# zxhuang1698/ShapeClipper

Measured on AMD Instinct MI355X. Metric: train-step images/sec (Pix3D cfg, bs32/GPU), higher is better.
Workload: dtype f32 (bf16x3-split MFMA, fp32 accumulate)

## Files before the change

### shapeclipper_amd/csrc/bn_act.hip

```cpp
#include <hip/hip_runtime.h>
#include <stdlib.h>
#include <stdint.h>
#include <type_traits>

namespace sc {

constexpr int BN_T = 256;

template <int W> struct Vec;
template <> struct Vec<4> {
    float v[4];
    __device__ __forceinline__ static Vec ld(const float* p) {
        const float4 t = *reinterpret_cast<const float4*>(p);
        return Vec{{t.x, t.y, t.z, t.w}};
    }
    __device__ __forceinline__ void st(float* p) const { *reinterpret_cast<float4*>(p) = make_float4(v[0], v[1], v[2], v[3]); }
};
template <> struct Vec<1> {
    float v[1];
    __device__ __forceinline__ static Vec ld(const float* p) { return Vec{{*p}}; }
    __device__ __forceinline__ void st(float* p) const { *p = v[0]; }
};

struct BnShare {
    int g, s, S, n0, Ng;
};
__device__ __forceinline__ BnShare bn_share(int N, int G) {
    BnShare sh;
    sh.S = gridDim.y / G;
    sh.g = blockIdx.y / sh.S;
    sh.s = blockIdx.y - sh.g * sh.S;
    sh.Ng = N / G;
    sh.n0 = sh.g * sh.Ng;
    return sh;
}

template <class F>
__device__ __forceinline__ void bn_iterate(const BnShare& sh, int C, int HW, int c, F&& f) {
    const int cnt = (sh.Ng - sh.s + sh.S - 1) / sh.S;
    if ((HW & 3) == 0) {
        const int hw4 = HW >> 2, total = cnt * hw4;
#pragma unroll 2
        for (int idx = threadIdx.x; idx < total; idx += BN_T) {
            const int nl = idx / hw4, i = idx - nl * hw4;
            f(((size_t)(sh.n0 + sh.s + nl * sh.S) * C + c) * HW + 4 * i, std::integral_constant<int, 4>{});
        }
    } else {
        const int total = cnt * HW;
        for (int idx = threadIdx.x; idx < total; idx += BN_T) {
            const int nl = idx / HW, i = idx - nl * HW;
            f(((size_t)(sh.n0 + sh.s + nl * sh.S) * C + c) * HW + i, std::integral_constant<int, 1>{});
        }
    }
}

__device__ __forceinline__ void block_sum2(float& a, float& b, float* red) {
    for (int d = 32; d >= 1; d >>= 1) {
        a += __shfl_xor(a, d);
        b += __shfl_xor(b, d);
    }
    const int w = threadIdx.x >> 6;
    __syncthreads();
    if ((threadIdx.x & 63) == 0) {
        red[w] = a;
        red[BN_T / 64 + w] = b;
    }
    __syncthreads();
    a = 0.f;
    b = 0.f;
    for (int k = 0; k < BN_T / 64; ++k) {
        a += red[k];
        b += red[BN_T / 64 + k];
    }
}

__device__ __forceinline__ void combine_partials(const float* partial, int c, int g, int S, int G, float& a, float& b) {
    a = 0.f;
    b = 0.f;
    const float* p = partial + ((size_t)c * G * S + (size_t)g * S) * 2;
    for (int k = 0; k < S; ++k) {
        a += p[2 * k];
        b += p[2 * k + 1];
    }
}

__device__ __forceinline__ void store_partial(float* partial, int c, const BnShare& sh, int G, float a, float b) {
    float* p = partial + ((size_t)c * G * sh.S + (size_t)sh.g * sh.S + sh.s) * 2;
    p[0] = a;
    p[1] = b;
}

__global__ __launch_bounds__(BN_T) void bn_stats_kernel(const float* __restrict__ x, int N, int C, int HW, int G,
                                                        float* __restrict__ partial) {
    __shared__ float red[2 * BN_T / 64];
    const int c = blockIdx.x;
    const BnShare sh = bn_share(N, G);
    const float K = x[((size_t)sh.n0 * C + c) * HW];
    float s1 = 0.f, s2 = 0.f;
    bn_iterate(sh, C, HW, c, [&](size_t off, auto w) {
        const auto v = Vec<decltype(w)::value>::ld(x + off);
#pragma unroll
        for (int k = 0; k < decltype(w)::value; ++k) {
            const float d = v.v[k] - K;
            s1 += d;
            s2 += d * d;
        }
    });
    block_sum2(s1, s2, red);
    if (threadIdx.x == 0) store_partial(partial, c, sh, G, s1, s2);
}

struct BnStatArgs {
    const float* x; const float* partial;
    float* save_mean; float* save_rstd;
    float* run_mean; float* run_var; int64_t* n_tracked;
    int N, C, HW, G, training;
    float eps, momentum;
};

__device__ __forceinline__ void bn_forward_stats(const BnStatArgs& a, int c, const BnShare& sh, float& mean, float& rstd) {
    const float n = (float)sh.Ng * (float)a.HW;
    auto group_stats = [&](int g, float& m, float& var) {
        float s1, s2;
        combine_partials(a.partial, c, g, sh.S, a.G, s1, s2);
        const float dm = s1 / n;
        const float v0 = s2 / n - dm * dm;
        var = v0 < 0.f ? 0.f : v0;
        m = a.x[((size_t)g * sh.Ng * a.C + c) * a.HW] + dm;
    };
    if (a.training) {
        float var;
        group_stats(sh.g, mean, var);
        rstd = rsqrtf(var + a.eps);
    } else {
        mean = a.run_mean[c];
        rstd = rsqrtf(a.run_var[c] + a.eps);
    }
    if (blockIdx.y == 0 && threadIdx.x == 0) {
        for (int g = 0; g < a.G; ++g) {
            float m = mean, r = rstd;
            if (a.training) {
                float var;
                group_stats(g, m, var);
                r = rsqrtf(var + a.eps);
                if (a.run_mean) {
                    a.run_mean[c] = (1.f - a.momentum) * a.run_mean[c] + a.momentum * m;
                    a.run_var[c] = (1.f - a.momentum) * a.run_var[c] + a.momentum * (n > 1.f ? var * n / (n - 1.f) : var);
                }
            }
            a.save_mean[(size_t)g * a.C + c] = m;
            a.save_rstd[(size_t)g * a.C + c] = r;
        }
        if (a.training && a.n_tracked && c == 0) *a.n_tracked += a.G;
    }
}

struct BnFwdArgs {
    BnStatArgs st;
    const float* res; const float* gamma; const float* beta; float* y;
    int relu;
};

__global__ __launch_bounds__(BN_T) void bn_apply_fwd_kernel(BnFwdArgs a) {
    const int c = blockIdx.x;
    const BnShare sh = bn_share(a.st.N, a.st.G);
    float mean, rstd;
    bn_forward_stats(a.st, c, sh, mean, rstd);
    const float scale = a.gamma[c] * rstd, shift = a.beta[c] - mean * scale;
    const float* x = a.st.x;
    bn_iterate(sh, a.st.C, a.st.HW, c, [&](size_t off, auto w) {
        constexpr int W = decltype(w)::value;
        auto v = Vec<W>::ld(x + off);
        if (a.res) {
            const auto r = Vec<W>::ld(a.res + off);
#pragma unroll
            for (int k = 0; k < W; ++k) v.v[k] = fmaf(v.v[k], scale, shift) + r.v[k];
        } else {
#pragma unroll
            for (int k = 0; k < W; ++k) v.v[k] = fmaf(v.v[k], scale, shift);
        }
        if (a.relu) {
#pragma unroll
            for (int k = 0; k < W; ++k) v.v[k] = v.v[k] < 0.f ? 0.f : v.v[k];
        }
        v.st(a.y + off);
    });
}

struct BnBwdArgs {
    const float* dy; const float* x; const float* y;
    const float* gamma; const float* beta; const float* mean; const float* rstd;
    float* partial; float* dx; float* dres; float* dgamma; float* dbeta;
    int N, C, HW, G, relu, training, has_res;
};

template <int W>
__device__ __forceinline__ Vec<W> bn_masked_grad(const BnBwdArgs& a, size_t off, const Vec<W>& xv, float scale, float shift) {
    auto g = Vec<W>::ld(a.dy + off);
    if (a.relu) {
        if (a.has_res) {
            const auto yv = Vec<W>::ld(a.y + off);
#pragma unroll
            for (int k = 0; k < W; ++k) g.v[k] = yv.v[k] <= 0.f ? 0.f : g.v[k];
        } else {
#pragma unroll
            for (int k = 0; k < W; ++k) g.v[k] = fmaf(xv.v[k], scale, shift) <= 0.f ? 0.f : g.v[k];
        }
    }
    return g;
}

__global__ __launch_bounds__(BN_T) void bn_bwd_stats_kernel(BnBwdArgs a) {
    __shared__ float red[2 * BN_T / 64];
    const int c = blockIdx.x;
    const BnShare sh = bn_share(a.N, a.G);
    const float mean = a.mean[(size_t)sh.g * a.C + c], rstd = a.rstd[(size_t)sh.g * a.C + c];
    const float scale = a.gamma[c] * rstd, shift = a.beta[c] - mean * scale;
    float s1 = 0.f, s2 = 0.f;
    bn_iterate(sh, a.C, a.HW, c, [&](size_t off, auto w) {
        constexpr int W = decltype(w)::value;
        const auto xv = Vec<W>::ld(a.x + off);
        const auto g = bn_masked_grad<W>(a, off, xv, scale, shift);
#pragma unroll
        for (int k = 0; k < W; ++k) {
            s1 += g.v[k];
            s2 += g.v[k] * ((xv.v[k] - mean) * rstd);
        }
        if (a.dres) g.st(a.dres + off);
    });
    block_sum2(s1, s2, red);
    if (threadIdx.x == 0) store_partial(a.partial, c, sh, a.G, s1, s2);
}

__global__ __launch_bounds__(BN_T) void bn_bwd_apply_kernel(BnBwdArgs a) {
    const int c = blockIdx.x;
    const BnShare sh = bn_share(a.N, a.G);
    const float mean = a.mean[(size_t)sh.g * a.C + c], rstd = a.rstd[(size_t)sh.g * a.C + c], gamma = a.gamma[c];
    const float scale = gamma * rstd, shift = a.beta[c] - mean * scale;
    float sg, sgx;
    combine_partials(a.partial, c, sh.g, sh.S, a.G, sg, sgx);
    if (blockIdx.y == 0 && threadIdx.x == 0) {
        float tg = 0.f, tgx = 0.f;
        for (int g = 0; g < a.G; ++g) {
            float u, v;
            combine_partials(a.partial, c, g, sh.S, a.G, u, v);
            tg += u;
            tgx += v;
        }
        a.dgamma[c] = tgx;
        a.dbeta[c] = tg;
    }
    if (!a.dx) return;
    const float n = (float)sh.Ng * (float)a.HW;
    const float mg = a.training ? sg / n : 0.f, mgx = a.training ? sgx / n : 0.f;
    bn_iterate(sh, a.C, a.HW, c, [&](size_t off, auto w) {
        constexpr int W = decltype(w)::value;
        const auto xv = Vec<W>::ld(a.x + off);
        const auto g = a.dres ? Vec<W>::ld(a.dres + off) : bn_masked_grad<W>(a, off, xv, scale, shift);
        Vec<W> o;
#pragma unroll
        for (int k = 0; k < W; ++k) o.v[k] = scale * (g.v[k] - mg - (xv.v[k] - mean) * rstd * mgx);
        o.st(a.dx + off);
    });
}

struct PoolFwdArgs {
    BnStatArgs st;
    const float* gamma; const float* beta; float* y; int* idx;
    int H, W, Ho, Wo;
};

__global__ __launch_bounds__(BN_T) void bn_relu_pool_fwd_kernel(PoolFwdArgs a) {
    const int c = blockIdx.x;
    const BnShare sh = bn_share(a.st.N, a.st.G);
    const int HW = a.H * a.W, C = a.st.C;
    float mean, rstd;
    bn_forward_stats(a.st, c, sh, mean, rstd);
    const float scale = a.gamma[c] * rstd, shift = a.beta[c] - mean * scale;
    const int HoWo = a.Ho * a.Wo;
    const int cnt = (sh.Ng - sh.s + sh.S - 1) / sh.S, total = cnt * HoWo;
    for (int t = threadIdx.x; t < total; t += BN_T) {
        const int nl = t / HoWo, o = t - nl * HoWo;
        const int ho = o / a.Wo, wo = o - ho * a.Wo;
        const size_t plane = ((size_t)(sh.n0 + sh.s + nl * sh.S) * C + c);
        const float* xp = a.st.x + plane * HW;
        float best = -__builtin_inff();
        int bi = -1;
#pragma unroll
        for (int dh = 0; dh < 3; ++dh) {
            const int h = 2 * ho - 1 + dh;
            if (h < 0 || h >= a.H) continue;
#pragma unroll
            for (int dw = 0; dw < 3; ++dw) {
                const int w = 2 * wo - 1 + dw;
                if (w < 0 || w >= a.W) continue;
                const float u = fmaf(xp[h * a.W + w], scale, shift), v = u < 0.f ? 0.f : u;
                if (v > best || bi < 0 || v != v) {
                    best = v;
                    bi = h * a.W + w;
                }
            }
        }
        a.y[plane * HoWo + o] = best;
        a.idx[plane * HoWo + o] = bi;
    }
}

__global__ __launch_bounds__(BN_T) void bn_relu_pool_fwd2_kernel(PoolFwdArgs a) {
    const int c = blockIdx.x;
    const BnShare sh = bn_share(a.st.N, a.st.G);
    const int HW = a.H * a.W, C = a.st.C, W = a.W;
    float mean, rstd;
    bn_forward_stats(a.st, c, sh, mean, rstd);
    const float scale = a.gamma[c] * rstd, shift = a.beta[c] - mean * scale;
    const int HoWo = a.Ho * a.Wo;
    const int cnt = (sh.Ng - sh.s + sh.S - 1) / sh.S, total = cnt * HoWo;
    const int lane = threadIdx.x & 63;
    for (int t0 = 0; t0 < total; t0 += BN_T) {
        const int t = t0 + threadIdx.x;
        const bool on = t < total;
        const int tt = on ? t : total - 1;
        const int nl = tt / HoWo, o = tt - nl * HoWo;
        const int ho = o / a.Wo, wo = o - ho * a.Wo;
        const size_t plane = ((size_t)(sh.n0 + sh.s + nl * sh.S) * C + c);
        const float* xp = a.st.x + plane * HW;
        float best = -__builtin_inff();
        int bi = -1;
#pragma unroll
        for (int dh = 0; dh < 3; ++dh) {
            const int h = 2 * ho - 1 + dh;
            const bool hv = h >= 0 && h < a.H;
            float2 v = make_float2(0.f, 0.f);
            if (hv) v = *reinterpret_cast<const float2*>(xp + h * W + 2 * wo);
            const float u0 = fmaf(v.x, scale, shift), u1 = fmaf(v.y, scale, shift);
            const float r0 = u0 < 0.f ? 0.f : u0, r1 = u1 < 0.f ? 0.f : u1;
            float left = __shfl_up(r1, 1);
            if (lane == 0 && wo > 0 && hv) {
                const float ul = fmaf(xp[h * W + 2 * wo - 1], scale, shift);
                left = ul < 0.f ? 0.f : ul;
            }
            if (!hv) continue;
            if (wo > 0 && (left > best || bi < 0 || left != left)) { best = left; bi = h * W + 2 * wo - 1; }
            if (r0 > best || bi < 0 || r0 != r0) { best = r0; bi = h * W + 2 * wo; }
            if (r1 > best || bi < 0 || r1 != r1) { best = r1; bi = h * W + 2 * wo + 1; }
        }
        if (on) {
            a.y[plane * HoWo + o] = best;
            a.idx[plane * HoWo + o] = bi;
        }
    }
}

template <int R>
__global__ __launch_bounds__(BN_T) void bn_relu_pool_fwd_rows_kernel(PoolFwdArgs a) {
    const int c = blockIdx.x;
    const BnShare sh = bn_share(a.st.N, a.st.G);
    const int HW = a.H * a.W, C = a.st.C, W = a.W;
    float mean, rstd;
    bn_forward_stats(a.st, c, sh, mean, rstd);
    const float scale = a.gamma[c] * rstd, shift = a.beta[c] - mean * scale;
    const int HoWo = a.Ho * a.Wo;
    const int RG = (a.Ho + R - 1) / R, per = RG * a.Wo;
    const int cnt = (sh.Ng - sh.s + sh.S - 1) / sh.S, total = cnt * per;
    const int lane = threadIdx.x & 63;
    for (int t0 = 0; t0 < total; t0 += BN_T) {
        const int t = t0 + threadIdx.x;
        const bool on = t < total;
        const int tt = on ? t : total - 1;
        const int nl = tt / per, o = tt - nl * per;
        const int rg = o / a.Wo, wo = o - rg * a.Wo;
        const int ho0 = rg * R;
        const size_t plane = ((size_t)(sh.n0 + sh.s + nl * sh.S) * C + c);
        const float* xp = a.st.x + plane * HW;
        float2 v[2 * R + 1];
        float lf[2 * R + 1];
#pragma unroll
        for (int k = 0; k < 2 * R + 1; ++k) {
            const int h = 2 * ho0 - 1 + k;
            const bool hv = h >= 0 && h < a.H;
            v[k] = make_float2(0.f, 0.f);
            lf[k] = 0.f;
            if (hv) v[k] = *reinterpret_cast<const float2*>(xp + h * W + 2 * wo);
            if (lane == 0 && wo > 0 && hv) lf[k] = xp[h * W + 2 * wo - 1];
        }
        float r0[2 * R + 1], r1[2 * R + 1], left[2 * R + 1];
#pragma unroll
        for (int k = 0; k < 2 * R + 1; ++k) {
            const float u0 = fmaf(v[k].x, scale, shift), u1 = fmaf(v[k].y, scale, shift);
            r0[k] = u0 < 0.f ? 0.f : u0;
            r1[k] = u1 < 0.f ? 0.f : u1;
            left[k] = __shfl_up(r1[k], 1);
            if (lane == 0) {
                const float ul = fmaf(lf[k], scale, shift);
                left[k] = ul < 0.f ? 0.f : ul;
            }
        }
#pragma unroll
        for (int r = 0; r < R; ++r) {
            const int ho = ho0 + r;
            float best = -__builtin_inff();
            int bi = -1;
#pragma unroll
            for (int dh = 0; dh < 3; ++dh) {
                const int k = 2 * r + dh, h = 2 * ho - 1 + dh;
                if (h < 0 || h >= a.H) continue;
                if (wo > 0 && (left[k] > best || bi < 0 || left[k] != left[k])) { best = left[k]; bi = h * W + 2 * wo - 1; }
                if (r0[k] > best || bi < 0 || r0[k] != r0[k]) { best = r0[k]; bi = h * W + 2 * wo; }
                if (r1[k] > best || bi < 0 || r1[k] != r1[k]) { best = r1[k]; bi = h * W + 2 * wo + 1; }
            }
            if (on && ho < a.Ho) {
                a.y[plane * HoWo + ho * a.Wo + wo] = best;
                a.idx[plane * HoWo + ho * a.Wo + wo] = bi;
            }
        }
    }
}

struct PoolBwdArgs {
    const float* dy; const int* idx; const float* x; const float* gamma; const float* beta; const float* mean;
    const float* rstd; float* partial; float* dx;
    int N, C, H, W, Ho, Wo, G;
    float* dgamma; float* dbeta;
    int training;
};

template <bool V2, int MODE>
__global__ __launch_bounds__(BN_T) void bn_relu_pool_bwd_gather_kernel(PoolBwdArgs a) {
    __shared__ float red[2 * BN_T / 64];
    const int c = blockIdx.x;
    const BnShare sh = bn_share(a.N, a.G);
    const int HW = a.H * a.W, HoWo = a.Ho * a.Wo;
    const int Hq = (a.H + 1) >> 1, Wq = (a.W + 1) >> 1, Q = Hq * Wq;
    const float mean = a.mean[(size_t)sh.g * a.C + c], rstd = a.rstd[(size_t)sh.g * a.C + c];
    const float scale = a.gamma[c] * rstd, shift = a.beta[c] - mean * scale;
    float sg = 0.f, sgx = 0.f;
    float mg = 0.f, mgx = 0.f;
    if (MODE == 2) {
        float tsg, tsgx;
        combine_partials(a.partial, c, sh.g, sh.S, a.G, tsg, tsgx);
        if (blockIdx.y == 0 && threadIdx.x == 0) {
            float tg = 0.f, tgx = 0.f;
            for (int g = 0; g < a.G; ++g) {
                float u, v;
                combine_partials(a.partial, c, g, sh.S, a.G, u, v);
                tg += u;
                tgx += v;
            }
            a.dgamma[c] = tgx;
            a.dbeta[c] = tg;
        }
        const float n = (float)sh.Ng * (float)HW;
        mg = a.training ? tsg / n : 0.f;
        mgx = a.training ? tsgx / n : 0.f;
    }
    const int cnt = (sh.Ng - sh.s + sh.S - 1) / sh.S, total = cnt * Q;
    for (int t = threadIdx.x; t < total; t += BN_T) {
        const int nl = t / Q, q = t - nl * Q;
        const int i = q / Wq, j = q - i * Wq;
        const size_t plane = ((size_t)(sh.n0 + sh.s + nl * sh.S) * a.C + c);
        int wi[2][2];
        float wd[2][2];
#pragma unroll
        for (int di = 0; di < 2; ++di)
#pragma unroll
            for (int dj = 0; dj < 2; ++dj) {
                const bool ok = (i + di) < a.Ho && (j + dj) < a.Wo;
                const size_t o = plane * HoWo + (size_t)(i + di) * a.Wo + (j + dj);
                wi[di][dj] = ok ? a.idx[o] : -1;
                wd[di][dj] = ok ? a.dy[o] : 0.f;
            }
#pragma unroll
        for (int eh = 0; eh < 2; ++eh) {
            const int h = 2 * i + eh;
            if (h >= a.H) continue;
            float2 xrow = make_float2(0.f, 0.f), grow;
            if (V2) xrow = *reinterpret_cast<const float2*>(a.x + plane * HW + h * a.W + 2 * j);
#pragma unroll
            for (int ew = 0; ew < 2; ++ew) {
                const int w = 2 * j + ew;
                if (w >= a.W) continue;
                const int pos = h * a.W + w;
                const float xv = V2 ? (ew ? xrow.y : xrow.x) : a.x[plane * HW + pos];
                float g = 0.f;
#pragma unroll
                for (int di = 0; di <= eh; ++di)
#pragma unroll
                    for (int dj = 0; dj <= ew; ++dj)
                        if (wi[di][dj] == pos) g += wd[di][dj];
                if (!(fmaf(xv, scale, shift) > 0.f)) g = 0.f;
                const float o = MODE == 2 ? scale * (g - mg - (xv - mean) * rstd * mgx) : g;
                if (V2) { if (ew) grow.y = o; else grow.x = o; }
                else if (MODE != 1) a.dx[plane * HW + pos] = o;
                sg += g;
                sgx += g * ((xv - mean) * rstd);
            }
            if (V2 && MODE != 1) *reinterpret_cast<float2*>(a.dx + plane * HW + h * a.W + 2 * j) = grow;
        }
    }
    if (MODE == 2) return;
    block_sum2(sg, sgx, red);
    if (threadIdx.x == 0) store_partial(a.partial, c, sh, a.G, sg, sgx);
}

template <int MODE, int R>
__global__ __launch_bounds__(BN_T) void bn_relu_pool_bwd_rows_kernel(PoolBwdArgs a) {
    __shared__ float red[2 * BN_T / 64];
    const int c = blockIdx.x;
    const BnShare sh = bn_share(a.N, a.G);
    const int HW = a.H * a.W, HoWo = a.Ho * a.Wo;
    const int Hq = (a.H + 1) >> 1, Wq = a.W >> 1, RG = (Hq + R - 1) / R, Q = RG * Wq;
    const float mean = a.mean[(size_t)sh.g * a.C + c], rstd = a.rstd[(size_t)sh.g * a.C + c];
    const float scale = a.gamma[c] * rstd, shift = a.beta[c] - mean * scale;
    float sg = 0.f, sgx = 0.f;
    float mg = 0.f, mgx = 0.f;
    if (MODE == 2) {
        float tsg, tsgx;
        combine_partials(a.partial, c, sh.g, sh.S, a.G, tsg, tsgx);
        if (blockIdx.y == 0 && threadIdx.x == 0) {
            float tg = 0.f, tgx = 0.f;
            for (int g = 0; g < a.G; ++g) {
                float u, v;
                combine_partials(a.partial, c, g, sh.S, a.G, u, v);
                tg += u;
                tgx += v;
            }
            a.dgamma[c] = tgx;
            a.dbeta[c] = tg;
        }
        const float n = (float)sh.Ng * (float)HW;
        mg = a.training ? tsg / n : 0.f;
        mgx = a.training ? tsgx / n : 0.f;
    }
    const int cnt = (sh.Ng - sh.s + sh.S - 1) / sh.S, total = cnt * Q;
    const int lane = threadIdx.x & 63;
    for (int t0 = 0; t0 < total; t0 += BN_T) {
        const int t = t0 + threadIdx.x;
        const bool on = t < total;
        const int tt = on ? t : total - 1;
        const int nl = tt / Q, q = tt - nl * Q;
        const int rg = q / Wq, j = q - rg * Wq, i0 = rg * R;
        const size_t plane = ((size_t)(sh.n0 + sh.s + nl * sh.S) * a.C + c);
        int wi[R + 1][2];
        float wd[R + 1][2];
        float2 xrow[2 * R];
        const bool own_right = lane == 63 && (j + 1) < a.Wo;
#pragma unroll
        for (int di = 0; di <= R; ++di) {
            const bool okr = (i0 + di) < a.Ho;
            const size_t o = plane * HoWo + (size_t)(i0 + di) * a.Wo + j;
            wi[di][0] = okr && j < a.Wo ? a.idx[o] : -1;
            wd[di][0] = okr && j < a.Wo ? a.dy[o] : 0.f;
            wi[di][1] = okr && own_right ? a.idx[o + 1] : -1;
            wd[di][1] = okr && own_right ? a.dy[o + 1] : 0.f;
        }
#pragma unroll
        for (int k = 0; k < 2 * R; ++k) {
            const int h = 2 * i0 + k;
            xrow[k] = h < a.H ? *reinterpret_cast<const float2*>(a.x + plane * HW + h * a.W + 2 * j) : make_float2(0.f, 0.f);
        }
#pragma unroll
        for (int di = 0; di <= R; ++di) {
            const int ri = __shfl_down(wi[di][0], 1);
            const float rd = __shfl_down(wd[di][0], 1);
            if (lane != 63) {
                const bool okc = (j + 1) < a.Wo;
                wi[di][1] = okc ? ri : -1;
                wd[di][1] = okc ? rd : 0.f;
            }
        }
#pragma unroll
        for (int r = 0; r < R; ++r) {
#pragma unroll
            for (int eh = 0; eh < 2; ++eh) {
                const int h = 2 * (i0 + r) + eh;
                if (h >= a.H) continue;
                float2 grow;
#pragma unroll
                for (int ew = 0; ew < 2; ++ew) {
                    const int pos = h * a.W + 2 * j + ew;
                    const float xv = ew ? xrow[2 * r + eh].y : xrow[2 * r + eh].x;
                    float g = 0.f;
#pragma unroll
                    for (int di = 0; di <= eh; ++di)
#pragma unroll
                        for (int dj = 0; dj <= ew; ++dj)
                            if (wi[r + di][dj] == pos) g += wd[r + di][dj];
                    if (!(fmaf(xv, scale, shift) > 0.f)) g = 0.f;
                    const float o = MODE == 2 ? scale * (g - mg - (xv - mean) * rstd * mgx) : g;
                    if (ew) grow.y = o; else grow.x = o;
                    if (on) {
                        sg += g;
                        sgx += g * ((xv - mean) * rstd);
                    }
                }
                if (MODE == 2 && on) *reinterpret_cast<float2*>(a.dx + plane * HW + h * a.W + 2 * j) = grow;
            }
        }
    }
    if (MODE == 2) return;
    block_sum2(sg, sgx, red);
    if (threadIdx.x == 0) store_partial(a.partial, c, sh, a.G, sg, sgx);
}

constexpr int BNF_T = 512, BNF_V = 10, BNF_G = 4;

template <int NV>
__device__ __forceinline__ void block_sum_f(float (&v)[NV], float* red) {
#pragma unroll
    for (int k = 0; k < NV; ++k)
        for (int d = 32; d >= 1; d >>= 1) v[k] += __shfl_xor(v[k], d);
    const int w = threadIdx.x >> 6;
    __syncthreads();
    if ((threadIdx.x & 63) == 0) {
#pragma unroll
        for (int k = 0; k < NV; ++k) red[k * (BNF_T / 64) + w] = v[k];
    }
    __syncthreads();
#pragma unroll
    for (int k = 0; k < NV; ++k) {
        float t = 0.f;
        for (int j = 0; j < BNF_T / 64; ++j) t += red[k * (BNF_T / 64) + j];
        v[k] = t;
    }
}

template <int W>
__device__ __forceinline__ bool bnf_slot(int j, int N, int C, int HW, int Ng, int c, size_t& off, int& g) {
    const int per = HW / W, idx = threadIdx.x + j * BNF_T;
    if (idx >= N * per) return false;
    const int n = idx / per, i = idx - n * per;
    off = ((size_t)n * C + c) * HW + (size_t)W * i;
    g = n / Ng;
    return true;
}

template <int W>
__global__ __launch_bounds__(BNF_T) void bn_fused_fwd_kernel(BnFwdArgs a) {
    __shared__ float red[2 * BNF_G * BNF_T / 64];
    const int c = blockIdx.x, C = a.st.C, HW = a.st.HW, G = a.st.G, N = a.st.N, Ng = N / G;
    const float n = (float)Ng * (float)HW;
    const float* x = a.st.x;
    const float gamma = a.gamma[c], beta = a.beta[c];
    Vec<W> xv[BNF_V];
    size_t off[BNF_V];
    int grp[BNF_V];
#pragma unroll
    for (int j = 0; j < BNF_V; ++j) {
        grp[j] = -1;
        if (bnf_slot<W>(j, N, C, HW, Ng, c, off[j], grp[j])) xv[j] = Vec<W>::ld(x + off[j]);
    }
    float mean[BNF_G], rstd[BNF_G];
    if (a.st.training) {
        float K[BNF_G], s[2 * BNF_G];
#pragma unroll
        for (int g = 0; g < BNF_G; ++g) {
            K[g] = g < G ? x[((size_t)g * Ng * C + c) * HW] : 0.f;
            s[2 * g] = 0.f;
            s[2 * g + 1] = 0.f;
        }
#pragma unroll
        for (int j = 0; j < BNF_V; ++j)
#pragma unroll
            for (int g = 0; g < BNF_G; ++g)
                if (grp[j] == g) {
#pragma unroll
                    for (int k = 0; k < W; ++k) {
                        const float d = xv[j].v[k] - K[g];
                        s[2 * g] += d;
                        s[2 * g + 1] += d * d;
                    }
                }
        block_sum_f(s, red);
#pragma unroll
        for (int g = 0; g < BNF_G; ++g) {
            const float dm = s[2 * g] / n, v0 = s[2 * g + 1] / n - dm * dm;
            const float var = v0 < 0.f ? 0.f : v0;
            mean[g] = K[g] + dm;
            rstd[g] = rsqrtf(var + a.st.eps);
            if (g < G && threadIdx.x == 0 && a.st.run_mean) {
                a.st.run_mean[c] = (1.f - a.st.momentum) * a.st.run_mean[c] + a.st.momentum * mean[g];
                a.st.run_var[c] = (1.f - a.st.momentum) * a.st.run_var[c] + a.st.momentum * (n > 1.f ? var * n / (n - 1.f) : var);
            }
        }
    } else {
#pragma unroll
        for (int g = 0; g < BNF_G; ++g) {
            mean[g] = a.st.run_mean[c];
            rstd[g] = rsqrtf(a.st.run_var[c] + a.st.eps);
        }
    }
    if (threadIdx.x == 0) {
        for (int g = 0; g < G; ++g) {
            a.st.save_mean[(size_t)g * C + c] = mean[g < BNF_G ? g : 0];
            a.st.save_rstd[(size_t)g * C + c] = rstd[g < BNF_G ? g : 0];
        }
        if (a.st.training && a.st.n_tracked && c == 0) *a.st.n_tracked += G;
    }
#pragma unroll
    for (int j = 0; j < BNF_V; ++j) {
        if (grp[j] < 0) continue;
        float m = mean[0], r = rstd[0];
#pragma unroll
        for (int g = 1; g < BNF_G; ++g)
            if (grp[j] == g) { m = mean[g]; r = rstd[g]; }
        const float scale = gamma * r, shift = beta - m * scale;
        Vec<W> v = xv[j];
        if (a.res) {
            const auto rv = Vec<W>::ld(a.res + off[j]);
#pragma unroll
            for (int k = 0; k < W; ++k) v.v[k] = fmaf(v.v[k], scale, shift) + rv.v[k];
        } else {
#pragma unroll
            for (int k = 0; k < W; ++k) v.v[k] = fmaf(v.v[k], scale, shift);
        }
        if (a.relu) {
#pragma unroll
            for (int k = 0; k < W; ++k) v.v[k] = v.v[k] < 0.f ? 0.f : v.v[k];
        }
        v.st(a.y + off[j]);
    }
}

template <int W>
__global__ __launch_bounds__(BNF_T) void bn_fused_bwd_kernel(BnBwdArgs a) {
    __shared__ float red[2 * BNF_G * BNF_T / 64];
    const int c = blockIdx.x, C = a.C, HW = a.HW, G = a.G, N = a.N, Ng = N / G;
    const float n = (float)Ng * (float)HW;
    const float gamma = a.gamma[c], beta = a.beta[c];
    float mean[BNF_G], rstd[BNF_G];
#pragma unroll
    for (int g = 0; g < BNF_G; ++g) {
        mean[g] = a.mean[(size_t)(g < G ? g : 0) * C + c];
        rstd[g] = a.rstd[(size_t)(g < G ? g : 0) * C + c];
    }
    Vec<W> xh[BNF_V], gr[BNF_V];
    size_t off[BNF_V];
    int grp[BNF_V];
    float s[2 * BNF_G];
#pragma unroll
    for (int g = 0; g < 2 * BNF_G; ++g) s[g] = 0.f;
#pragma unroll
    for (int j = 0; j < BNF_V; ++j) {
        grp[j] = -1;
        if (!bnf_slot<W>(j, N, C, HW, Ng, c, off[j], grp[j])) continue;
        float m = mean[0], r = rstd[0];
#pragma unroll
        for (int g = 1; g < BNF_G; ++g)
            if (grp[j] == g) { m = mean[g]; r = rstd[g]; }
        const float scale = gamma * r, shift = beta - m * scale;
        const auto xv = Vec<W>::ld(a.x + off[j]);
        gr[j] = bn_masked_grad<W>(a, off[j], xv, scale, shift);
        if (a.dres) gr[j].st(a.dres + off[j]);
#pragma unroll
        for (int k = 0; k < W; ++k) xh[j].v[k] = (xv.v[k] - m) * r;
#pragma unroll
        for (int g = 0; g < BNF_G; ++g)
            if (grp[j] == g) {
#pragma unroll
                for (int k = 0; k < W; ++k) {
                    s[2 * g] += gr[j].v[k];
                    s[2 * g + 1] += gr[j].v[k] * xh[j].v[k];
                }
            }
    }
    block_sum_f(s, red);
    if (threadIdx.x == 0) {
        float tg = 0.f, tgx = 0.f;
#pragma unroll
        for (int g = 0; g < BNF_G; ++g)
            if (g < G) { tg += s[2 * g]; tgx += s[2 * g + 1]; }
        a.dgamma[c] = tgx;
        a.dbeta[c] = tg;
    }
    if (!a.dx) return;
#pragma unroll
    for (int j = 0; j < BNF_V; ++j) {
        if (grp[j] < 0) continue;
        float r = rstd[0], sg = s[0], sgx = s[1];
#pragma unroll
        for (int g = 1; g < BNF_G; ++g)
            if (grp[j] == g) { r = rstd[g]; sg = s[2 * g]; sgx = s[2 * g + 1]; }
        const float scale = gamma * r, mg = a.training ? sg / n : 0.f, mgx = a.training ? sgx / n : 0.f;
        Vec<W> o;
#pragma unroll
        for (int k = 0; k < W; ++k) o.v[k] = scale * (gr[j].v[k] - mg - xh[j].v[k] * mgx);
        o.st(a.dx + off[j]);
    }
}

static inline bool bn_fused_takes(int N, int C, int HW, int G) {
#ifdef SC_BN_NO_FUSED
    return false;
#endif
    const long long vecs = (HW & 3) ? (long long)N * HW : (long long)N * (HW >> 2);
    return C >= 256 && G <= BNF_G && vecs <= (long long)BNF_T * BNF_V;
}

static inline int bn_splits(int Ng, int C, int G) {
    int S = (2048 + C * G - 1) / (C * G);
    if (S > Ng) S = Ng;
    if (S > 32) S = 32;
    return S < 1 ? 1 : S;
}

}

static inline bool bn_bad(int N, int C, int HW, int G) { return G < 1 || N % G != 0; }

extern "C" int sc_bn_splits(int N, int C) { return sc::bn_splits(N, C, 1); }

extern "C" int sc_bn_act_forward(const float* x, const float* res, const float* gamma, const float* beta, float* y,
                                 float* save_mean, float* save_rstd, float* run_mean, float* run_var,
                                 int64_t* n_tracked, float* partial, int N, int C, int HW, int relu, int training,
                                 int groups, float eps, float momentum, void* stream_) {
    if (N <= 0 || C <= 0 || HW <= 0) return 0;
    if (bn_bad(N, C, HW, groups)) return (int)hipErrorInvalidValue;
    hipStream_t st = (hipStream_t)stream_;
    sc::BnFwdArgs a{{x, partial, save_mean, save_rstd, run_mean, run_var, n_tracked, N, C, HW, groups, training, eps, momentum},
                    res, gamma, beta, y, relu};
    if (sc::bn_fused_takes(N, C, HW, groups)) {
        if (HW & 3) hipLaunchKernelGGL(sc::bn_fused_fwd_kernel<1>, dim3(C), dim3(sc::BNF_T), 0, st, a);
        else hipLaunchKernelGGL(sc::bn_fused_fwd_kernel<4>, dim3(C), dim3(sc::BNF_T), 0, st, a);
        return (int)hipGetLastError();
    }
    const dim3 grid(C, groups * sc::bn_splits(N / groups, C, groups));
    if (training) hipLaunchKernelGGL(sc::bn_stats_kernel, grid, dim3(sc::BN_T), 0, st, x, N, C, HW, groups, partial);
    hipLaunchKernelGGL(sc::bn_apply_fwd_kernel, grid, dim3(sc::BN_T), 0, st, a);
    return (int)hipGetLastError();
}

extern "C" int sc_bn_act_backward(const float* dy, const float* x, const float* y, const float* gamma,
                                  const float* beta, const float* mean, const float* rstd, float* partial, float* dx,
                                  float* dres, float* dgamma, float* dbeta, int N, int C, int HW, int relu,
                                  int training, int groups, void* stream_) {
    if (N <= 0 || C <= 0 || HW <= 0) return 0;
    if (bn_bad(N, C, HW, groups)) return (int)hipErrorInvalidValue;
    hipStream_t st = (hipStream_t)stream_;
    sc::BnBwdArgs a{dy, x, y, gamma, beta, mean, rstd, partial, dx, dres, dgamma, dbeta, N, C, HW, groups, relu, training,
                    (y != nullptr) ? 1 : 0};
    if (sc::bn_fused_takes(N, C, HW, groups)) {
        if (HW & 3) hipLaunchKernelGGL(sc::bn_fused_bwd_kernel<1>, dim3(C), dim3(sc::BNF_T), 0, st, a);
        else hipLaunchKernelGGL(sc::bn_fused_bwd_kernel<4>, dim3(C), dim3(sc::BNF_T), 0, st, a);
        return (int)hipGetLastError();
    }
    const dim3 grid(C, groups * sc::bn_splits(N / groups, C, groups));
    hipLaunchKernelGGL(sc::bn_bwd_stats_kernel, grid, dim3(sc::BN_T), 0, st, a);
    hipLaunchKernelGGL(sc::bn_bwd_apply_kernel, grid, dim3(sc::BN_T), 0, st, a);
    return (int)hipGetLastError();
}

extern "C" int sc_bn_relu_pool_forward(const float* x, const float* gamma, const float* beta, float* y, int* idx,
                                       float* save_mean, float* save_rstd, float* run_mean, float* run_var,
                                       int64_t* n_tracked, float* partial, int N, int C, int H, int W, int training,
                                       int groups, float eps, float momentum, void* stream_) {
    if (N <= 0 || C <= 0 || H <= 0 || W <= 0) return 0;
    if (bn_bad(N, C, H * W, groups)) return (int)hipErrorInvalidValue;
    hipStream_t st = (hipStream_t)stream_;
    const dim3 grid(C, groups * sc::bn_splits(N / groups, C, groups));
    if (training) hipLaunchKernelGGL(sc::bn_stats_kernel, grid, dim3(sc::BN_T), 0, st, x, N, C, H * W, groups, partial);
    sc::PoolFwdArgs a{{x, partial, save_mean, save_rstd, run_mean, run_var, n_tracked, N, C, H * W, groups, training, eps, momentum},
                      gamma, beta, y, idx, H, W, (H + 2 - 3) / 2 + 1, (W + 2 - 3) / 2 + 1};
#ifndef SC_POOL_ROWS
#define SC_POOL_ROWS 4
#endif
    if ((W & 1) == 0 && SC_POOL_ROWS > 0) hipLaunchKernelGGL(sc::bn_relu_pool_fwd_rows_kernel<(SC_POOL_ROWS > 0 ? SC_POOL_ROWS : 1)>, grid, dim3(sc::BN_T), 0, st, a);
    else if ((W & 1) == 0) hipLaunchKernelGGL(sc::bn_relu_pool_fwd2_kernel, grid, dim3(sc::BN_T), 0, st, a);
    else hipLaunchKernelGGL(sc::bn_relu_pool_fwd_kernel, grid, dim3(sc::BN_T), 0, st, a);
    return (int)hipGetLastError();
}

extern "C" int sc_bn_relu_pool_backward(const float* dy, const int* idx, const float* x, const float* gamma,
                                        const float* beta, const float* mean, const float* rstd, float* partial,
                                        float* dx, float* dgamma, float* dbeta, int N, int C, int H, int W,
                                        int training, int groups, void* stream_) {
    if (N <= 0 || C <= 0 || H <= 0 || W <= 0) return 0;
    if (bn_bad(N, C, H * W, groups)) return (int)hipErrorInvalidValue;
    hipStream_t st = (hipStream_t)stream_;
    const dim3 grid(C, groups * sc::bn_splits(N / groups, C, groups));
    sc::PoolBwdArgs a{dy, idx, x, gamma, beta, mean, rstd, partial, dx, N, C, H, W, (H + 2 - 3) / 2 + 1, (W + 2 - 3) / 2 + 1, groups, dgamma, dbeta, training};
#ifndef SC_POOL_BWD_ROWS
#define SC_POOL_BWD_ROWS 1
#endif
    if ((W & 1) == 0 && SC_POOL_BWD_ROWS > 0) {
        hipLaunchKernelGGL((sc::bn_relu_pool_bwd_rows_kernel<1, (SC_POOL_BWD_ROWS > 0 ? SC_POOL_BWD_ROWS : 1)>), grid, dim3(sc::BN_T), 0, st, a);
        hipLaunchKernelGGL((sc::bn_relu_pool_bwd_rows_kernel<2, (SC_POOL_BWD_ROWS > 0 ? SC_POOL_BWD_ROWS : 1)>), grid, dim3(sc::BN_T), 0, st, a);
        return (int)hipGetLastError();
    }
    if ((W & 1) == 0) {
        hipLaunchKernelGGL((sc::bn_relu_pool_bwd_gather_kernel<true, 1>), grid, dim3(sc::BN_T), 0, st, a);
        hipLaunchKernelGGL((sc::bn_relu_pool_bwd_gather_kernel<true, 2>), grid, dim3(sc::BN_T), 0, st, a);
        return (int)hipGetLastError();
    }
    hipLaunchKernelGGL((sc::bn_relu_pool_bwd_gather_kernel<false, 0>), grid, dim3(sc::BN_T), 0, st, a);
    sc::BnBwdArgs b{nullptr, x, nullptr, gamma, beta, mean, rstd, partial, dx, dx, dgamma, dbeta, N, C, H * W, groups, 0, training, 0};
    hipLaunchKernelGGL(sc::bn_bwd_apply_kernel, grid, dim3(sc::BN_T), 0, st, b);
    return (int)hipGetLastError();
}
```

Baseline: 1015.

## Extend single-launch fused batchnorm to mid-size layers with 1024-thread blocks

Adds a mid-size single-kernel batchnorm forward/backward path (1024 threads, register-resident tiles) for layers with C>=128 and HW divisible by 4, so they no longer need separate stats and apply launches. The fused kernels are restructured: an incremental index walker with 32-bit byte offsets replaces per-slot divisions and 64-bit offsets. Per-group partial sums are kept in running registers and parked in shared memory instead of per-group branch accumulation, and the block reduction is spread across threads with a readfirstlane broadcast. This raises register and LDS pressure and relies on 32-bit offsets, which a new size guard protects.

```diff
diff --git a/shapeclipper_amd/csrc/bn_act.hip b/shapeclipper_amd/csrc/bn_act.hip
--- a/shapeclipper_amd/csrc/bn_act.hip
+++ b/shapeclipper_amd/csrc/bn_act.hip
@@ -195,11 +195,11 @@
 };
 
 template <int W>
-__device__ __forceinline__ Vec<W> bn_masked_grad(const BnBwdArgs& a, size_t off, const Vec<W>& xv, float scale, float shift) {
-    auto g = Vec<W>::ld(a.dy + off);
+__device__ __forceinline__ Vec<W> bn_masked_grad(const BnBwdArgs& a, const float* dy, const float* y, const Vec<W>& xv, float scale, float shift) {
+    auto g = Vec<W>::ld(dy);
     if (a.relu) {
         if (a.has_res) {
-            const auto yv = Vec<W>::ld(a.y + off);
+            const auto yv = Vec<W>::ld(y);
 #pragma unroll
             for (int k = 0; k < W; ++k) g.v[k] = yv.v[k] <= 0.f ? 0.f : g.v[k];
         } else {
@@ -220,7 +220,7 @@
     bn_iterate(sh, a.C, a.HW, c, [&](size_t off, auto w) {
         constexpr int W = decltype(w)::value;
         const auto xv = Vec<W>::ld(a.x + off);
-        const auto g = bn_masked_grad<W>(a, off, xv, scale, shift);
+        const auto g = bn_masked_grad<W>(a, a.dy + off, a.y + off, xv, scale, shift);
 #pragma unroll
         for (int k = 0; k < W; ++k) {
             s1 += g.v[k];
@@ -256,7 +256,7 @@
     bn_iterate(sh, a.C, a.HW, c, [&](size_t off, auto w) {
         constexpr int W = decltype(w)::value;
         const auto xv = Vec<W>::ld(a.x + off);
-        const auto g = a.dres ? Vec<W>::ld(a.dres + off) : bn_masked_grad<W>(a, off, xv, scale, shift);
+        const auto g = a.dres ? Vec<W>::ld(a.dres + off) : bn_masked_grad<W>(a, a.dy + off, a.y + off, xv, scale, shift);
         Vec<W> o;
 #pragma unroll
         for (int k = 0; k < W; ++k) o.v[k] = scale * (g.v[k] - mg - (xv.v[k] - mean) * rstd * mgx);
@@ -603,74 +603,124 @@
 }
 
 constexpr int BNF_T = 512, BNF_V = 10, BNF_G = 4;
-
-template <int NV>
-__device__ __forceinline__ void block_sum_f(float (&v)[NV], float* red) {
-#pragma unroll
-    for (int k = 0; k < NV; ++k)
-        for (int d = 32; d >= 1; d >>= 1) v[k] += __shfl_xor(v[k], d);
+constexpr int BNM_T = 1024, BNM_VF = 19, BNM_VB = 13;
+
+template <int T, int NV>
+__device__ __forceinline__ void block_sum_f(const float* col, float (&v)[NV], float* red) {
     const int w = threadIdx.x >> 6;
+#pragma unroll
+    for (int k = 0; k < NV; ++k) {
+        float t = col[k * T];
+        for (int d = 32; d >= 1; d >>= 1) t += __shfl_xor(t, d);
+        if ((threadIdx.x & 63) == 0) red[k * (T / 64) + w] = t;
+        __builtin_amdgcn_sched_barrier(0);
+    }
     __syncthreads();
-    if ((threadIdx.x & 63) == 0) {
-#pragma unroll
-        for (int k = 0; k < NV; ++k) red[k * (BNF_T / 64) + w] = v[k];
+    if (threadIdx.x < NV) {
+        float t = 0.f;
+        for (int j = 0; j < T / 64; ++j) t += red[threadIdx.x * (T / 64) + j];
+        red[NV * (T / 64) + threadIdx.x] = t;
     }
     __syncthreads();
 #pragma unroll
-    for (int k = 0; k < NV; ++k) {
-        float t = 0.f;
-        for (int j = 0; j < BNF_T / 64; ++j) t += red[k * (BNF_T / 64) + j];
-        v[k] = t;
-    }
-}
-
-template <int W>
-__device__ __forceinline__ bool bnf_slot(int j, int N, int C, int HW, int Ng, int c, size_t& off, int& g) {
-    const int per = HW / W, idx = threadIdx.x + j * BNF_T;
-    if (idx >= N * per) return false;
-    const int n = idx / per, i = idx - n * per;
-    off = ((size_t)n * C + c) * HW + (size_t)W * i;
-    g = n / Ng;
-    return true;
-}
-
-template <int W>
-__global__ __launch_bounds__(BNF_T) void bn_fused_fwd_kernel(BnFwdArgs a) {
-    __shared__ float red[2 * BNF_G * BNF_T / 64];
+    for (int k = 0; k < NV; ++k) v[k] = __builtin_bit_cast(float, __builtin_amdgcn_readfirstlane(__builtin_bit_cast(int, red[NV * (T / 64) + k])));
+}
+
+template <int W, int T>
+struct BnfWalk {
+    int n, i, per, dn, di, N, Ng;
+    __device__ __forceinline__ BnfWalk(int N_, int HW, int Ng_) : N(N_), Ng(Ng_) {
+        int t = threadIdx.x;
+        asm volatile("" : "+v"(t));
+        per = HW / W;
+        n = t / per, i = t - n * per;
+        dn = T / per, di = T - dn * per;
+    }
+    __device__ __forceinline__ bool valid() const { return n < N; }
+    __device__ __forceinline__ unsigned off(int C, int HW, int c) const { return (((unsigned)n * C + c) * HW + (unsigned)W * i) * 4u; }
+    __device__ __forceinline__ int group() const { return (n >= Ng) + (n >= 2 * Ng) + (n >= 3 * Ng); }
+    __device__ __forceinline__ void next() {
+        n += dn, i += di;
+        if (i >= per) i -= per, ++n;
+        asm volatile("" : "+v"(n), "+v"(i));
+    }
+};
+static_assert(BNF_G == 4, "BnfWalk::group() counts three group boundaries");
+template <class P>
+__device__ __forceinline__ P* bnf_at(P* base, unsigned byte_off) {
+    using B = std::conditional_t<std::is_const<P>::value, const char, char>;
+    return reinterpret_cast<P*>(reinterpret_cast<B*>(base) + byte_off);
+}
+template <int EVERY = 4>
+__device__ __forceinline__ void bnf_sched_fence(int j) {
+    if (j % EVERY == EVERY - 1) __builtin_amdgcn_sched_barrier(0);
+}
+
+template <int T>
+struct BnfSums {
+    float* park;
+    float c1 = 0.f, c2 = 0.f;
+    int gc = 0;
+    __device__ __forceinline__ explicit BnfSums(float* park_) : park(park_ + threadIdx.x) {
+#pragma unroll
+        for (int k = 0; k < 2 * BNF_G; ++k) park[k * T] = 0.f;
+    }
+    __device__ __forceinline__ void enter(int g_new) {
+        const bool sw = g_new != gc;
+        c1 = sw ? 0.f : c1;
+        c2 = sw ? 0.f : c2;
+        gc = g_new;
+        asm volatile("" : "+v"(c1), "+v"(c2), "+v"(gc));
+    }
+    __device__ __forceinline__ void leave() {
+        park[2 * gc * T] = c1;
+        park[(2 * gc + 1) * T] = c2;
+    }
+};
+
+template <int W, int T, int V>
+__global__ __launch_bounds__(T) void bn_fused_fwd_kernel(BnFwdArgs a) {
+    __shared__ float red[2 * BNF_G * (T / 64 + 1)], park[2 * BNF_G * T];
     const int c = blockIdx.x, C = a.st.C, HW = a.st.HW, G = a.st.G, N = a.st.N, Ng = N / G;
     const float n = (float)Ng * (float)HW;
     const float* x = a.st.x;
     const float gamma = a.gamma[c], beta = a.beta[c];
-    Vec<W> xv[BNF_V];
-    size_t off[BNF_V];
-    int grp[BNF_V];
-#pragma unroll
-    for (int j = 0; j < BNF_V; ++j) {
-        grp[j] = -1;
-        if (bnf_slot<W>(j, N, C, HW, Ng, c, off[j], grp[j])) xv[j] = Vec<W>::ld(x + off[j]);
+    const unsigned off0 = (unsigned)c * HW * 4u;
+    Vec<W> xv[V];
+    {
+        BnfWalk<W, T> wk(N, HW, Ng);
+#pragma unroll
+        for (int j = 0; j < V; ++j) {
+            xv[j] = Vec<W>::ld(bnf_at(x, wk.valid() ? wk.off(C, HW, c) : off0));
+            wk.next();
+            bnf_sched_fence(j);
+        }
     }
     float mean[BNF_G], rstd[BNF_G];
     if (a.st.training) {
-        float K[BNF_G], s[2 * BNF_G];
-#pragma unroll
-        for (int g = 0; g < BNF_G; ++g) {
-            K[g] = g < G ? x[((size_t)g * Ng * C + c) * HW] : 0.f;
-            s[2 * g] = 0.f;
-            s[2 * g + 1] = 0.f;
-        }
-#pragma unroll
-        for (int j = 0; j < BNF_V; ++j)
-#pragma unroll
-            for (int g = 0; g < BNF_G; ++g)
-                if (grp[j] == g) {
-#pragma unroll
-                    for (int k = 0; k < W; ++k) {
-                        const float d = xv[j].v[k] - K[g];
-                        s[2 * g] += d;
-                        s[2 * g + 1] += d * d;
-                    }
-                }
-        block_sum_f(s, red);
+        float K[BNF_G];
+#pragma unroll
+        for (int g = 0; g < BNF_G; ++g) K[g] = g < G ? x[((size_t)g * Ng * C + c) * HW] : 0.f;
+        BnfSums<T> t(park);
+        BnfWalk<W, T> wk(N, HW, Ng);
+#pragma unroll
+        for (int j = 0; j < V; ++j) {
+            const bool on = wk.valid();
+            t.enter(on ? wk.group() : t.gc);
+            float Kc = K[0];
+#pragma unroll
+            for (int g = 1; g < BNF_G; ++g) Kc = t.gc == g ? K[g] : Kc;
+#pragma unroll
+            for (int k = 0; k < W; ++k) {
+                const float d = on ? xv[j].v[k] - Kc : 0.f;
+                t.c1 += d;
+                t.c2 += d * d;
+            }
+            t.leave();
+            wk.next();
+        }
+        float s[2 * BNF_G];
+        block_sum_f<T>(t.park, s, red);
 #pragma unroll
         for (int g = 0; g < BNF_G; ++g) {
             const float dm = s[2 * g] / n, v0 = s[2 * g + 1] / n - dm * dm;
@@ -690,23 +740,28 @@
         }
     }
     if (threadIdx.x == 0) {
-        for (int g = 0; g < G; ++g) {
-            a.st.save_mean[(size_t)g * C + c] = mean[g < BNF_G ? g : 0];
-            a.st.save_rstd[(size_t)g * C + c] = rstd[g < BNF_G ? g : 0];
-        }
+#pragma unroll
+        for (int g = 0; g < BNF_G; ++g)
+            if (g < G) {
+                a.st.save_mean[(size_t)g * C + c] = mean[g];
+                a.st.save_rstd[(size_t)g * C + c] = rstd[g];
+            }
         if (a.st.training && a.st.n_tracked && c == 0) *a.st.n_tracked += G;
     }
-#pragma unroll
-    for (int j = 0; j < BNF_V; ++j) {
-        if (grp[j] < 0) continue;
+    BnfWalk<W, T> wk(N, HW, Ng);
+#pragma unroll
+    for (int j = 0; j < V; ++j) {
+        const bool on = wk.valid();
+        const int gj = wk.group();
+        const unsigned off = on ? wk.off(C, HW, c) : off0;
         float m = mean[0], r = rstd[0];
 #pragma unroll
         for (int g = 1; g < BNF_G; ++g)
-            if (grp[j] == g) { m = mean[g]; r = rstd[g]; }
+            if (gj == g) { m = mean[g]; r = rstd[g]; }
         const float scale = gamma * r, shift = beta - m * scale;
         Vec<W> v = xv[j];
         if (a.res) {
-            const auto rv = Vec<W>::ld(a.res + off[j]);
+            const auto rv = Vec<W>::ld(bnf_at(a.res, off));
 #pragma unroll
             for (int k = 0; k < W; ++k) v.v[k] = fmaf(v.v[k], scale, shift) + rv.v[k];
         } else {
@@ -717,53 +772,56 @@
 #pragma unroll
             for (int k = 0; k < W; ++k) v.v[k] = v.v[k] < 0.f ? 0.f : v.v[k];
         }
-        v.st(a.y + off[j]);
-    }
-}
-
-template <int W>
-__global__ __launch_bounds__(BNF_T) void bn_fused_bwd_kernel(BnBwdArgs a) {
-    __shared__ float red[2 * BNF_G * BNF_T / 64];
+        if (on) v.st(bnf_at(a.y, off));
+        wk.next();
+        bnf_sched_fence(j);
+    }
+}
+
+template <int W, int T, int V>
+__global__ __launch_bounds__(T) void bn_fused_bwd_kernel(BnBwdArgs a) {
+    __shared__ float red[2 * BNF_G * (T / 64 + 1)], park[2 * BNF_G * T];
     const int c = blockIdx.x, C = a.C, HW = a.HW, G = a.G, N = a.N, Ng = N / G;
     const float n = (float)Ng * (float)HW;
     const float gamma = a.gamma[c], beta = a.beta[c];
+    const unsigned off0 = (unsigned)c * HW * 4u;
     float mean[BNF_G], rstd[BNF_G];
 #pragma unroll
     for (int g = 0; g < BNF_G; ++g) {
         mean[g] = a.mean[(size_t)(g < G ? g : 0) * C + c];
         rstd[g] = a.rstd[(size_t)(g < G ? g : 0) * C + c];
     }
-    Vec<W> xh[BNF_V], gr[BNF_V];
-    size_t off[BNF_V];
-    int grp[BNF_V];
+    Vec<W> xh[V], gr[V];
+    BnfSums<T> t(park);
+    {
+        BnfWalk<W, T> wk(N, HW, Ng);
+#pragma unroll
+        for (int j = 0; j < V; ++j) {
+            const bool on = wk.valid();
+            t.enter(on ? wk.group() : t.gc);
+            const unsigned off = on ? wk.off(C, HW, c) : off0;
+            float m = mean[0], r = rstd[0];
+#pragma unroll
+            for (int g = 1; g < BNF_G; ++g)
+                if (t.gc == g) { m = mean[g]; r = rstd[g]; }
+            const float scale = gamma * r, shift = beta - m * scale;
+            const auto xv = Vec<W>::ld(bnf_at(a.x, off));
+            gr[j] = bn_masked_grad<W>(a, bnf_at(a.dy, off), bnf_at(a.y, off), xv, scale, shift);
+            if (a.dres && on) gr[j].st(bnf_at(a.dres, off));
+#pragma unroll
+            for (int k = 0; k < W; ++k) {
+                xh[j].v[k] = (xv.v[k] - m) * r;
+                const float gk = on ? gr[j].v[k] : 0.f, xk = on ? xh[j].v[k] : 0.f;
+                t.c1 += gk;
+                t.c2 += gk * xk;
+            }
+            t.leave();
+            wk.next();
+            bnf_sched_fence<2>(j);
+        }
+    }
     float s[2 * BNF_G];
-#pragma unroll
-    for (int g = 0; g < 2 * BNF_G; ++g) s[g] = 0.f;
-#pragma unroll
-    for (int j = 0; j < BNF_V; ++j) {
-        grp[j] = -1;
-        if (!bnf_slot<W>(j, N, C, HW, Ng, c, off[j], grp[j])) continue;
-        float m = mean[0], r = rstd[0];
-#pragma unroll
-        for (int g = 1; g < BNF_G; ++g)
-            if (grp[j] == g) { m = mean[g]; r = rstd[g]; }
-        const float scale = gamma * r, shift = beta - m * scale;
-        const auto xv = Vec<W>::ld(a.x + off[j]);
-        gr[j] = bn_masked_grad<W>(a, off[j], xv, scale, shift);
-        if (a.dres) gr[j].st(a.dres + off[j]);
-#pragma unroll
-        for (int k = 0; k < W; ++k) xh[j].v[k] = (xv.v[k] - m) * r;
-#pragma unroll
-        for (int g = 0; g < BNF_G; ++g)
-            if (grp[j] == g) {
-#pragma unroll
-                for (int k = 0; k < W; ++k) {
-                    s[2 * g] += gr[j].v[k];
-                    s[2 * g + 1] += gr[j].v[k] * xh[j].v[k];
-                }
-            }
-    }
-    block_sum_f(s, red);
+    block_sum_f<T>(t.park, s, red);
     if (threadIdx.x == 0) {
         float tg = 0.f, tgx = 0.f;
 #pragma unroll
@@ -773,27 +831,37 @@
         a.dbeta[c] = tg;
     }
     if (!a.dx) return;
-#pragma unroll
-    for (int j = 0; j < BNF_V; ++j) {
-        if (grp[j] < 0) continue;
+    BnfWalk<W, T> wk(N, HW, Ng);
+#pragma unroll
+    for (int j = 0; j < V; ++j) {
+        const bool on = wk.valid();
+        const int gj = wk.group();
         float r = rstd[0], sg = s[0], sgx = s[1];
 #pragma unroll
         for (int g = 1; g < BNF_G; ++g)
-            if (grp[j] == g) { r = rstd[g]; sg = s[2 * g]; sgx = s[2 * g + 1]; }
+            if (gj == g) { r = rstd[g]; sg = s[2 * g]; sgx = s[2 * g + 1]; }
         const float scale = gamma * r, mg = a.training ? sg / n : 0.f, mgx = a.training ? sgx / n : 0.f;
         Vec<W> o;
 #pragma unroll
         for (int k = 0; k < W; ++k) o.v[k] = scale * (gr[j].v[k] - mg - xh[j].v[k] * mgx);
-        o.st(a.dx + off[j]);
-    }
-}
-
-static inline bool bn_fused_takes(int N, int C, int HW, int G) {
+        if (on) o.st(bnf_at(a.dx, wk.off(C, HW, c)));
+        wk.next();
+        bnf_sched_fence(j);
+    }
+}
+
+enum BnForm { BN_TWO_LAUNCH = 0, BN_SMALL = 1, BN_MID = 2 };
+static inline BnForm bn_fused_takes(int N, int C, int HW, int G, bool backward) {
 #ifdef SC_BN_NO_FUSED
-    return false;
+    return BN_TWO_LAUNCH;
 #endif
     const long long vecs = (HW & 3) ? (long long)N * HW : (long long)N * (HW >> 2);
-    return C >= 256 && G <= BNF_G && vecs <= (long long)BNF_T * BNF_V;
+    if (G > BNF_G || (long long)N * C * HW * 4 >= (1LL << 32)) return BN_TWO_LAUNCH;
+    if (C >= 256 && vecs <= (long long)BNF_T * BNF_V) return BN_SMALL;
+#ifndef SC_BN_NO_MID
+    if (C >= 128 && (HW & 3) == 0 && vecs <= (long long)BNM_T * (backward ? BNM_VB : BNM_VF)) return BN_MID;
+#endif
+    return BN_TWO_LAUNCH;
 }
 
 static inline int bn_splits(int Ng, int C, int G) {
@@ -818,9 +886,14 @@
     hipStream_t st = (hipStream_t)stream_;
     sc::BnFwdArgs a{{x, partial, save_mean, save_rstd, run_mean, run_var, n_tracked, N, C, HW, groups, training, eps, momentum},
                     res, gamma, beta, y, relu};
-    if (sc::bn_fused_takes(N, C, HW, groups)) {
-        if (HW & 3) hipLaunchKernelGGL(sc::bn_fused_fwd_kernel<1>, dim3(C), dim3(sc::BNF_T), 0, st, a);
-        else hipLaunchKernelGGL(sc::bn_fused_fwd_kernel<4>, dim3(C), dim3(sc::BNF_T), 0, st, a);
+    const sc::BnForm form = sc::bn_fused_takes(N, C, HW, groups, false);
+    if (form == sc::BN_SMALL) {
+        if (HW & 3) hipLaunchKernelGGL((sc::bn_fused_fwd_kernel<1, sc::BNF_T, sc::BNF_V>), dim3(C), dim3(sc::BNF_T), 0, st, a);
+        else hipLaunchKernelGGL((sc::bn_fused_fwd_kernel<4, sc::BNF_T, sc::BNF_V>), dim3(C), dim3(sc::BNF_T), 0, st, a);
+        return (int)hipGetLastError();
+    }
+    if (form == sc::BN_MID) {
+        hipLaunchKernelGGL((sc::bn_fused_fwd_kernel<4, sc::BNM_T, sc::BNM_VF>), dim3(C), dim3(sc::BNM_T), 0, st, a);
         return (int)hipGetLastError();
     }
     const dim3 grid(C, groups * sc::bn_splits(N / groups, C, groups));
@@ -838,9 +911,14 @@
     hipStream_t st = (hipStream_t)stream_;
     sc::BnBwdArgs a{dy, x, y, gamma, beta, mean, rstd, partial, dx, dres, dgamma, dbeta, N, C, HW, groups, relu, training,
                     (y != nullptr) ? 1 : 0};
-    if (sc::bn_fused_takes(N, C, HW, groups)) {
-        if (HW & 3) hipLaunchKernelGGL(sc::bn_fused_bwd_kernel<1>, dim3(C), dim3(sc::BNF_T), 0, st, a);
-        else hipLaunchKernelGGL(sc::bn_fused_bwd_kernel<4>, dim3(C), dim3(sc::BNF_T), 0, st, a);
+    const sc::BnForm form = sc::bn_fused_takes(N, C, HW, groups, true);
+    if (form == sc::BN_SMALL) {
+        if (HW & 3) hipLaunchKernelGGL((sc::bn_fused_bwd_kernel<1, sc::BNF_T, sc::BNF_V>), dim3(C), dim3(sc::BNF_T), 0, st, a);
+        else hipLaunchKernelGGL((sc::bn_fused_bwd_kernel<4, sc::BNF_T, sc::BNF_V>), dim3(C), dim3(sc::BNF_T), 0, st, a);
+        return (int)hipGetLastError();
+    }
+    if (form == sc::BN_MID) {
+        hipLaunchKernelGGL((sc::bn_fused_bwd_kernel<4, sc::BNM_T, sc::BNM_VB>), dim3(C), dim3(sc::BNM_T), 0, st, a);
         return (int)hipGetLastError();
     }
     const dim3 grid(C, groups * sc::bn_splits(N / groups, C, groups));
```

After: 928.6. 0.915x the previous value.
